# EmreAdabag/osqp

Measured on AMD Instinct MI355X. Metric: ADMM iters/sec (single QP), higher is better.
Workload: dtype f64; 1 GPU; config2 random sparse QP n=10000 m=20000 nnzA=200000 nnzPtriu=59985, one step = osqp_update_rho(0.1) + cold-started osqp_solve; adaptive_rho_interval=100, status=solved, graph_launches=4775, resident_gave_up=0, resident_slow_waits=0, parallelism=replicas x1 (a single QP does not shard)

## Files before the change

osqp_amd/csrc/engine.hip:

```cpp
#include <hip/hip_runtime.h>
#include <cstdio>
#include <new>
#include <cstdlib>
#include <cstring>
#include <cmath>
#include <vector>
#include <map>
#include <algorithm>
#include <mutex>
#include <condition_variable>
#include <thread>
#include <atomic>
#include <chrono>
#include "../../include/osqp_amd_engine.h"

#define TB 256
#define MAX_CHUNK 2048
#define LONG_ROW 512
#define HUGE_ROW 8192
#define MAX_PARTS 1024
#define MAX_HUGE_FOLD 4
#define INF_BOUND 1e26

#define HIPCHK(call)                                                            \
  do {                                                                          \
    hipError_t _e = (call);                                                     \
    if (_e != hipSuccess) {                                                     \
      fprintf(stderr, "osqp_amd: HIP error %s at %s:%d (%s)\n",                 \
              hipGetErrorString(_e), __FILE__, __LINE__, #call);                \
      return HIPENG_ERR_HIP;                                                    \
    }                                                                           \
  } while (0)

struct RowBlk { int r0, r1, k0, k1; };
#define IS_LONG(b) ((b).r1 - (b).r0 == 1 && (b).k1 - (b).k0 >= LONG_ROW)
struct __attribute__((aligned(32))) G4 { double r, w, s, m; };

struct DevMat {
  int nrows, nblk;
  int nstream;
  int nwave;
  const int    *rowptr;
  const int    *col;
  const unsigned short *col16;
  const double *val;
  const int    *split;
  const RowBlk *blk;
};

#define DENSE_MAX 128
struct DenseBlk { int c0, b, off, pitch; };
struct DenseP {
  int nblk;
  const DenseBlk *blk;
  const double *val;
};

struct State {
  int    run;
  int    done;
  int    stalled;
  int    neg_curv;
  int    iters[2];
  int    neg_curv_seen;
  int    iters_last;
  int    iters_max;
  int    iters_min;
  int    forced;
  long long iters_total;
  long long admm_done;
  double rz[2];
  double tol2;
  double gam[2], alp[2];
  int    hist_r;
  long long admm_target;
  unsigned res_epoch;
  int    res_fail;
  int    res_pipe_off;
  int    res_chk_fail;
  int    res_dbg[4];
  int    res_slow;
  int    res_slow_max;
  int    res_repub;
  int    res_slow_hist[4];
  unsigned res_slow_xcc;
  int    res_slow_last[4];
};

struct Params {
  double sigma, alpha, eps_rel, eps_abs, cinv;
  int    pcg_max_iter, use_cvec, has_scaling, pad0;
  double ex_theta;
  int    ex_h0, ex_h1;
  int    no_restart;
};

struct Ctx {
  int n, m;
  DevMat A, M;
  DevMat Mk;
  DenseP dP;
  int nh, hrow[MAX_HUGE_FOLD];
  const double *hcol;
  int gridA, gridM;
  double *xy, *z, *zt, *va, *vb, *q, *l, *u, *rho, *rhoinv, *minv, *pdiag;
  double *r, *zz, *kp, *pt0, *pt1, *dxy, *dy, *cvec;
  double *init_r, *init_z;
  double *vx, *vold;
  double *pdir, *ut;
  G4     *g4;
  int     init_stride;
  int     fin_wave_rows;
  double *vd;
  int     plain_rhs;
  const int *plain_skip;
  const unsigned short *u0map;
  double *u0pos;
  int     nelim;
  const int *erow, *ecol, *epos;
  double *rhoe, *ecoef, *edinv, *xte;
  double *D, *Dinv, *E, *Einv;
  double *part_rz, *part_rr, *part_bb, *part_pkp, *part_s0, *part_s1, *part_s2, *part_gam, *part_del;
  const double *fin_rr;
  int fin_cnt;
  double *scal;
  double *part_h;
  State  *st;
  const Params *prm;
#ifdef OSQP_AMD_TIMELINE
  unsigned long long *tl;
#endif
};

#ifdef OSQP_AMD_TIMELINE
#define TL_CAP (1 << 20)
#define TL_MARK(c, id) do { if (blockIdx.x == 0 && threadIdx.x == 0) { const unsigned long long k_ = atomicAdd((c).tl, 1ull); \
    if (k_ < TL_CAP - 2) (c).tl[1 + k_] = ((unsigned long long)(id) << 56) | (wall_clock64() & 0x00FFFFFFFFFFFFFFull); } } while (0)
#else
#define TL_MARK(c, id) do { } while (0)
#endif

enum {
  SC_PRI_U, SC_PRI_S, SC_Z_U, SC_Z_S, SC_AX_U, SC_AX_S,
  SC_DUA_U, SC_DUA_S, SC_Q_U, SC_Q_S, SC_ATY_U, SC_ATY_S, SC_PX_U, SC_PX_S,
  SC_DYN_U, SC_DYN_S, SC_DXN_U, SC_DXN_S,
  SC_ATDY_U, SC_ATDY_S, SC_PDX_U, SC_PDX_S, SC_ADX_VIOL,
  SC_OBJ, SC_DYLHS, SC_QDX,
  SC_COUNT
};
#define SCI(x) ((x) * 16)

template <int CTRL>
__device__ __forceinline__ double dpp_move(double v) {
  int lo = __double2loint(v), hi = __double2hiint(v);
  lo = __builtin_amdgcn_mov_dpp(lo, CTRL, 0xF, 0xF, true); hi = __builtin_amdgcn_mov_dpp(hi, CTRL, 0xF, 0xF, true);
  return __hiloint2double(hi, lo);
}
__device__ __forceinline__ double lane_value(double v, int lane) {
  return __hiloint2double(__builtin_amdgcn_readlane(__double2hiint(v), lane), __builtin_amdgcn_readlane(__double2loint(v), lane));
}
__device__ __forceinline__ double wave_sum(double v) {
  v += dpp_move<0xB1>(v); v += dpp_move<0x4E>(v); v += dpp_move<0x141>(v); v += dpp_move<0x140>(v);
  return (lane_value(v, 0) + lane_value(v, 16)) + (lane_value(v, 32) + lane_value(v, 48));
}

__device__ __forceinline__ double block_sum(double v, double *red) {
  v = wave_sum(v);
  const int lane = threadIdx.x & 63, w = threadIdx.x >> 6;
  __syncthreads();
  if (lane == 0) red[w] = v;
  __syncthreads();
  if (threadIdx.x == 0) red[4] = (red[0] + red[1]) + (red[2] + red[3]);
  __syncthreads();
  return red[4];
}

__device__ __forceinline__ void block_sum3(double &a, double &b, double &c, double *red) {
  a = wave_sum(a); b = wave_sum(b); c = wave_sum(c);
  const int lane = threadIdx.x & 63, w = threadIdx.x >> 6;
  __syncthreads();
  if (lane == 0) { red[w] = a; red[4 + w] = b; red[8 + w] = c; }
  __syncthreads();
  a = (red[0] + red[1]) + (red[2] + red[3]);
  b = (red[4] + red[5]) + (red[6] + red[7]);
  c = (red[8] + red[9]) + (red[10] + red[11]);
}

template <int NA>
__device__ __forceinline__ void reduce_parts(const double *a0, const double *a1,
                                             const double *a2, int count,
                                             double *red, double out[NA]) {
  double s0 = 0, s1 = 0, s2 = 0;
  for (int i = threadIdx.x; i < count; i += TB) {
    s0 += a0[i];
    if (NA > 1) s1 += a1[i];
    if (NA > 2) s2 += a2[i];
  }
  if (NA == 1) { out[0] = block_sum(s0, red); return; }
  block_sum3(s0, s1, s2, red);
  out[0] = s0; out[1] = s1;
  if (NA > 2) out[2] = s2;
}

__device__ __forceinline__ void atomic_max_pos(double *slot, double v) {
  atomicMax(reinterpret_cast<unsigned long long *>(slot),
            static_cast<unsigned long long>(__double_as_longlong(v)));
}

__device__ __forceinline__ void block_max_to(double v, double *slot, double *red) {
#pragma unroll
  for (int off = 32; off > 0; off >>= 1) v = fmax(v, __shfl_down(v, off, 64));
  const int lane = threadIdx.x & 63, w = threadIdx.x >> 6;
  __syncthreads();
  if (lane == 0) red[w] = v;
  __syncthreads();
  if (threadIdx.x == 0) atomic_max_pos(slot, fmax(fmax(red[0], red[1]), fmax(red[2], red[3])));
}

template <int NV>
__device__ __forceinline__ void stage_products(const DevMat &Mx, const RowBlk b,
                                               const double *in0, const double *in1,
                                               double *l0, double *l1) {
  constexpr int E = MAX_CHUNK / TB;
  const int cnt = b.k1 - b.k0;
  int cc[E]; double vv[E], x0[E], x1[E];
#pragma unroll
  for (int e = 0; e < E; ++e) {
    const int k = threadIdx.x + e * TB;
    if (k < cnt) { cc[e] = Mx.col[b.k0 + k]; vv[e] = Mx.val[b.k0 + k]; }
  }
#pragma unroll
  for (int e = 0; e < E; ++e) {
    const int k = threadIdx.x + e * TB;
    if (k < cnt) { x0[e] = in0[cc[e]]; if (NV == 2) x1[e] = in1[cc[e]]; }
  }
#pragma unroll
  for (int e = 0; e < E; ++e) {
    const int k = threadIdx.x + e * TB;
    if (k < cnt) { l0[k] = vv[e] * x0[e]; if (NV == 2) l1[k] = vv[e] * x1[e]; }
  }
}

__device__ __forceinline__ double row_sum(const double *l, int a, int b) {
  double s = 0.0;
  for (int k = a; k < b; ++k) s += l[k];
  return s;
}

__device__ __forceinline__ double row_sum_par(const double *l, int a, int b, int lane, int L) {
  double s = 0.0;
  for (int k = a + lane; k < b; k += L) s += l[k];
  if (L >= 2) s += dpp_move<0xB1>(s);
  if (L >= 4) s += dpp_move<0x4E>(s);
  if (L >= 8) s += dpp_move<0x141>(s);
  if (L >= 16) s += dpp_move<0x140>(s);
  if (L >= 32) s += __shfl_xor(s, 16, 64);
  if (L == 64) s += __shfl_xor(s, 32, 64);
  return s;
}
__device__ __forceinline__ int lanes_for(int nrows) {
  int L = 64;
  while (L > 1 && L * nrows > TB) L >>= 1;
  return L;
}

__device__ __forceinline__ double long_row_dot(const DevMat &Mx, int ka, int kb,
                                               const double *in, double *red) {
  double s0 = 0.0, s1 = 0.0, s2 = 0.0, s3 = 0.0;
  int k = ka + threadIdx.x;
  for (; k + 3 * TB < kb; k += 4 * TB) {
    const int c0 = Mx.col[k], c1 = Mx.col[k + TB], c2 = Mx.col[k + 2 * TB], c3 = Mx.col[k + 3 * TB];
    const double v0 = Mx.val[k], v1 = Mx.val[k + TB], v2 = Mx.val[k + 2 * TB], v3 = Mx.val[k + 3 * TB];
    s0 += v0 * in[c0]; s1 += v1 * in[c1]; s2 += v2 * in[c2]; s3 += v3 * in[c3];
  }
  for (; k < kb; k += TB) s0 += Mx.val[k] * in[Mx.col[k]];
  return block_sum((s0 + s1) + (s2 + s3), red);
}

#define ROW_U 12
template <bool NARROW, class F>
__device__ __forceinline__ double wave_row_dot_t(const DevMat &Mx, int ka, int kb, F xval) {
  const int lane = threadIdx.x & 63;
  double s0 = 0.0, s1 = 0.0, s2 = 0.0, s3 = 0.0;
  for (int k0 = ka + lane; k0 - lane < kb; k0 += 64 * ROW_U) {
    int cc[ROW_U]; double vv[ROW_U], xx[ROW_U];
#pragma unroll
    for (int q = 0; q < ROW_U; ++q) {
      const int kc = min(k0 + 64 * q, kb - 1);
      cc[q] = NARROW ? (int)Mx.col16[kc] : Mx.col[kc];
      vv[q] = Mx.val[kc];
    }
#pragma unroll
    for (int q = 0; q < ROW_U; ++q) xx[q] = xval(cc[q]);
#pragma unroll
    for (int q = 0; q < ROW_U; ++q) if (k0 + 64 * q >= kb) vv[q] = 0.0;
#pragma unroll
    for (int q = 0; q < ROW_U; q += 4) { s0 += vv[q] * xx[q]; s1 += vv[q + 1] * xx[q + 1]; s2 += vv[q + 2] * xx[q + 2]; s3 += vv[q + 3] * xx[q + 3]; }
  }
  return wave_sum((s0 + s1) + (s2 + s3));
}
template <class F>
__device__ __forceinline__ double wave_row_dot(const DevMat &Mx, int ka, int kb, F xval) {
  return Mx.col16 ? wave_row_dot_t<true>(Mx, ka, kb, xval) : wave_row_dot_t<false>(Mx, ka, kb, xval);
}

template <bool EARLY = false, class XL>
__device__ __forceinline__ double dense_block_mv_x(const DenseP &dP, const DenseBlk d, XL xload, double *scratch) {
  const int lane = threadIdx.x & 63, w = threadIdx.x >> 6;
  const double2 *dv = reinterpret_cast<const double2 *>(dP.val + d.off);
  const int hp = d.pitch >> 1;
  double xe = 0.0;
  if (EARLY) {
    if ((int)threadIdx.x < d.b) xe = xload(d.c0 + (int)threadIdx.x);
    asm volatile("s_waitcnt vmcnt(0)" ::: "memory");
  }
  double2 v[DENSE_MAX / 4];
#pragma unroll
  for (int q = 0; q < DENSE_MAX / 4; ++q) {
    const int j = w + 4 * q;
    v[q] = (j < d.b && lane < hp) ? dv[(size_t)j * hp + lane] : double2{0.0, 0.0};
  }
  double *xl = scratch + 4 * DENSE_MAX;
  if ((int)threadIdx.x < DENSE_MAX) xl[threadIdx.x] = EARLY ? xe : ((int)threadIdx.x < d.b ? xload(d.c0 + (int)threadIdx.x) : 0.0);
  __syncthreads();
  double a0 = 0.0, a1 = 0.0;
#pragma unroll
  for (int q = 0; q < DENSE_MAX / 4; ++q) {
    const double u = xl[min(w + 4 * q, DENSE_MAX - 1)];
    a0 += v[q].x * u; a1 += v[q].y * u;
  }
  scratch[w * DENSE_MAX + 2 * lane] = a0; scratch[w * DENSE_MAX + 2 * lane + 1] = a1;
  __syncthreads();
  const int r = threadIdx.x;
  return r < d.b ? (scratch[r] + scratch[DENSE_MAX + r]) + (scratch[2 * DENSE_MAX + r] + scratch[3 * DENSE_MAX + r]) : 0.0;
}
__device__ __forceinline__ double dense_block_mv(const DenseP &dP, const DenseBlk d, const double *x, double *scratch) {
  return dense_block_mv_x<false>(dP, d, [x](int j) { return x[j]; }, scratch);
}

#define LDS_DECL(NV)                                   \
  __shared__ double lprod[(NV) * MAX_CHUNK];           \
  __shared__ double red[16]


__global__ void __launch_bounds__(TB) k_vd(Ctx c) {
  for (int k = blockIdx.x * TB + threadIdx.x; k < c.n + c.m; k += gridDim.x * TB) c.vd[k] = c.vb[k] - c.vx[k];
}
template <bool DENSE>
__global__ void __launch_bounds__(TB) k_pcg_init(Ctx c, int bench) {
  State *st = c.st;
  TL_MARK(c, 1);
  if (!bench) {
    if (st->stalled || st->res_fail) return;
    if (st->admm_done >= st->admm_target) { if (blockIdx.x == 0 && threadIdx.x == 0) st->run = 0; return; }
  }
  LDS_DECL(2);
  const Params prm = *c.prm;
  double prz = 0, prr = 0, pbb = 0;
  const DevMat &Mm = DENSE ? c.Mk : c.M;
  if (DENSE)
  for (int db = blockIdx.x; db < c.dP.nblk; db += gridDim.x) {
    const DenseBlk d = c.dP.blk[db];
    double sA = c.plain_rhs ? 0.0 : dense_block_mv(c.dP, d, c.vx, lprod);
    if ((int)threadIdx.x < d.b) {
      const int j = d.c0 + threadIdx.x;
      double sB = 0.0;
      if (c.plain_rhs) {
        for (int k = Mm.rowptr[j]; k < Mm.rowptr[j + 1]; ++k) { const int cc = Mm.col[k]; if (c.plain_skip && c.plain_skip[cc - c.n] >= 0) continue; sB += Mm.val[k] * c.vb[cc]; }
      } else {
        for (int k = Mm.rowptr[j]; k < Mm.rowptr[j + 1]; ++k) { const int cc = Mm.col[k]; const double v = Mm.val[k]; sA += v * c.vx[cc]; sB += v * c.vb[cc]; }
        for (int k = 0; k < c.nh; ++k) { const double hc = c.hcol[(size_t)k * c.n + j]; sA += hc * c.vx[c.n + c.hrow[k]]; sB += hc * c.vb[c.n + c.hrow[k]]; }
      }
      const double base = prm.use_cvec ? c.cvec[j] : (prm.sigma * c.xy[j] - c.q[j]);
      const double bj = base + sB;
      const double rj = c.plain_rhs ? bj : bj - prm.sigma * c.vx[j] - sA;
      const double zj = c.minv[j] * rj;
      c.init_r[(size_t)j * c.init_stride] = rj;
      c.init_z[j] = zj;
      if (c.u0pos) c.u0pos[c.u0map[j]] = zj;
      prz += rj * zj; prr += rj * rj; pbb += bj * bj;
    }
    __syncthreads();
  }
  auto row_start = [&](int j, double sA, double sB) {
    if (DENSE) for (int k = 0; k < c.nh; ++k) { const double hc = c.hcol[(size_t)k * c.n + j]; sA += hc * c.vx[c.n + c.hrow[k]]; sB += hc * c.vb[c.n + c.hrow[k]]; }
    const double base = prm.use_cvec ? c.cvec[j] : (prm.sigma * c.xy[j] - c.q[j]);
    const bool gone = c.nelim && c.erow[j] >= 0;
    const double bj = gone ? 0.0 : base + sB;
    const double rj = gone ? 0.0 : bj - prm.sigma * c.vx[j] - sA;
    const double zj = c.minv[j] * rj;
    c.init_r[(size_t)j * c.init_stride] = rj;
    c.init_z[j] = zj;
    if (c.u0pos) c.u0pos[c.u0map[j]] = zj;
    prz += rj * zj; prr += rj * rj; pbb += bj * bj;
  };
  for (int bi = blockIdx.x; bi < Mm.nstream; bi += gridDim.x) {
    const RowBlk b = Mm.blk[bi];
    stage_products<2>(Mm, b, c.vx, c.vb, lprod, lprod + MAX_CHUNK);
    __syncthreads();
    const int RL = lanes_for(b.r1 - b.r0), rg = threadIdx.x / RL, rlane = threadIdx.x % RL;
    for (int j = b.r0 + rg; j < b.r1; j += TB / RL) {
      const int a0 = Mm.rowptr[j] - b.k0, a1 = Mm.rowptr[j + 1] - b.k0;
      const double sA = row_sum_par(lprod, a0, a1, rlane, RL);
      const double sB = row_sum_par(lprod + MAX_CHUNK, a0, a1, rlane, RL);
      if (rlane == 0) row_start(j, sA, sB);
    }
    __syncthreads();
  }
  for (int bi = Mm.nstream + blockIdx.x * (TB / 64) + (threadIdx.x >> 6); bi < Mm.nblk; bi += gridDim.x * (TB / 64)) {
    const RowBlk lb = Mm.blk[bi];
    const int lane = threadIdx.x & 63;
    if (c.vd) {
      const double acc = wave_row_dot(Mm, lb.k0, lb.k1, [&](int cc) { return c.vd[cc]; });
      if (lane == 0) row_start(lb.r0, -acc, 0.0);
      continue;
    }
    double a0 = 0.0, a1 = 0.0, b0 = 0.0, b1 = 0.0;
    const bool narrow = Mm.col16 != nullptr;
    constexpr int UI = 8;
    for (int k0 = lb.k0 + lane; k0 - lane < lb.k1; k0 += 64 * UI) {
      int cc[UI]; double vv[UI], xa[UI], xb[UI];
#pragma unroll
      for (int q = 0; q < UI; ++q) {
        const int kc = min(k0 + 64 * q, lb.k1 - 1);
        cc[q] = narrow ? (int)Mm.col16[kc] : Mm.col[kc];
        vv[q] = Mm.val[kc];
      }
#pragma unroll
      for (int q = 0; q < UI; ++q) { xa[q] = c.vx[cc[q]]; xb[q] = c.vb[cc[q]]; }
#pragma unroll
      for (int q = 0; q < UI; ++q) if (k0 + 64 * q >= lb.k1) vv[q] = 0.0;
#pragma unroll
      for (int q = 0; q < UI; q += 2) { a0 += vv[q] * xa[q]; b0 += vv[q] * xb[q]; a1 += vv[q + 1] * xa[q + 1]; b1 += vv[q + 1] * xb[q + 1]; }
    }
    const double sA = wave_sum(a0 + a1), sB = wave_sum(b0 + b1);
    if (lane == 0) row_start(lb.r0, sA, sB);
  }
  block_sum3(prz, prr, pbb, red);
  if (threadIdx.x == 0) {
    c.part_rz[blockIdx.x] = prz; c.part_rr[blockIdx.x] = prr; c.part_bb[blockIdx.x] = pbb;
    if (blockIdx.x == 0) {
      st->run = 1; st->done = 0; st->neg_curv = 0; st->iters[0] = 0; st->iters[1] = 0;
      if (st->hist_r < (1 << 20)) st->hist_r += 1;
    }
  }
}

#define EPT (MAX_CHUNK / TB)

struct CgStep { double alpha, beta; bool first, stop, conv, bad; };
__device__ __forceinline__ CgStep cg_step(double rr, double gam, double del, double gam_old, double alp_old,
                                          double tol2, int iters_prev, int neg, const Params &prm, bool bench) {
  CgStep s;
  s.first = gam_old == 0.0;
  s.bad = false;
  if (s.first) { s.beta = 0.0; s.alpha = gam / del; }
  else {
    s.beta = gam / gam_old;
    const double den = del - s.beta * gam / alp_old;
    if (!(den > 0.0) && del > 0.0) {
      if (!prm.no_restart && rr <= 1e8 * tol2) { s.first = true; s.beta = 0.0; s.alpha = gam / del; }
      else { s.alpha = gam / den; s.bad = true; }
    } else s.alpha = gam / den;
  }
  if (bench) { s.beta = 0.5; s.alpha = 1e-3; s.bad = false; }
  s.conv = rr <= tol2;
  s.bad = s.bad || !(s.alpha > 0.0) || !(del > 0.0);
  s.stop = !bench && (s.conv || iters_prev >= prm.pcg_max_iter || neg || s.bad);
  return s;
}
__global__ void __launch_bounds__(TB) k_cg_A(Ctx c, int it, int flags) {
  State *st = c.st;
  TL_MARK(c, 2);
  const bool bench = flags & 4, upd_only = flags & 16, apply_only = flags & 32;
  const bool pre = (flags & 8) || apply_only;
  if (!bench && it >= (flags >> 8) && (it >= st->iters_last || st->stalled) && (!st->run || st->done)) return;
  const int stalled = st->stalled, run = st->run, done = st->done, neg = st->neg_curv;
  const int iters_prev = st->iters[(it + 1) & 1];
  const double tol2_old = st->tol2, gam_old = st->gam[(it + 1) & 1], alp_old = st->alp[(it + 1) & 1];
  const Params prm = *c.prm;
  const bool has_blk = (int)blockIdx.x < c.A.nstream;
  RowBlk b = {0, 0, 0, 0};
  if (has_blk) b = c.A.blk[blockIdx.x];
  const int cnt = b.k1 - b.k0;
  const bool small = has_blk;
  const G4 *gold = c.g4 + (size_t)((it + 1) & 1) * c.n;
  G4 *gnew = c.g4 + (size_t)(it & 1) * c.n;
  int ecol[EPT]; double eval[EPT], g0[EPT], g1[EPT], g2[EPT], g3[EPT];
  int RL = lanes_for(b.r1 - b.r0);
  int rg = threadIdx.x / RL, rlane = threadIdx.x % RL;
  int rp0 = 0, rp1 = 0;
  double prho = 0.0;
  if (small) {
    if (b.r0 + rg < b.r1) { rp0 = c.A.rowptr[b.r0 + rg]; rp1 = c.A.rowptr[b.r0 + rg + 1]; prho = c.rhoe[b.r0 + rg]; }
#pragma unroll
    for (int e = 0; e < EPT; ++e) {
      const int k = threadIdx.x + e * TB;
      if (k < cnt) { ecol[e] = c.A.col[b.k0 + k]; eval[e] = c.A.val[b.k0 + k]; }
    }
#pragma unroll
    for (int e = 0; e < EPT; ++e) {
      const int k = threadIdx.x + e * TB;
      if (k < cnt) {
        const int cc = ecol[e];
        if (pre) g0[e] = c.ut[cc];
        else { const G4 g = gold[cc]; g0[e] = g.r; g1[e] = g.w; g2[e] = g.s; g3[e] = g.m; }
      }
    }
  }
  double q0 = 0, q1 = 0, q2 = 0;
  if (!apply_only) {
    const double *a1 = pre ? c.part_bb : c.part_gam;
    for (int i = threadIdx.x; i < c.gridM; i += TB) { q0 += c.part_rr[i]; q1 += a1[i]; if (!pre) q2 += c.part_del[i]; }
  }
  const int j0 = blockIdx.x * TB + threadIdx.x;
  double o_u = 0, o_w = 0, o_p = 0, o_s = 0, o_r = 0, o_x = 0, o_m = 0;
  if (!pre && j0 < c.n) {
    const G4 g = gold[j0];
    o_u = c.ut[j0]; o_w = g.w; o_p = c.pdir[j0]; o_s = g.s; o_r = g.r; o_x = gam_old == 0.0 ? c.vx[j0] : c.va[j0]; o_m = g.m;
  }
  if (!bench && (!run || done || ((flags & 8) && stalled))) return;
  LDS_DECL(1);
  double sums[3];
  bool first = false;
  double alpha = 0.0, beta = 0.0, tol2 = tol2_old;
  sums[0] = q0; sums[1] = q1; sums[2] = q2;
  if (!apply_only) block_sum3(sums[0], sums[1], sums[2], red);
  if (apply_only) {
  } else if (pre) {
    tol2 = fmax(prm.eps_rel * prm.eps_rel * sums[1], prm.eps_abs * prm.eps_abs);
    if (!bench && sums[0] <= tol2) {
      if (blockIdx.x == 0 && threadIdx.x == 0) { st->done = 1; st->tol2 = tol2; }
      return;
    }
    if (blockIdx.x == 0 && threadIdx.x == 0) { st->tol2 = tol2; st->gam[1] = 0.0; st->alp[1] = 0.0; }
  } else {
    const double gam = sums[1];
    const bool fresh = gam_old == 0.0;
    const CgStep cs = cg_step(sums[0], gam, sums[2], gam_old, alp_old, tol2, iters_prev, neg, prm, bench);
    first = cs.first; alpha = cs.alpha; beta = cs.beta;
    if (cs.stop) {
      if (blockIdx.x == 0 && threadIdx.x == 0) { st->done = cs.conv ? 1 : 2; if (cs.bad && !cs.conv) st->neg_curv = 1; }
      return;
    }
    if (blockIdx.x == 0 && threadIdx.x == 0) {
      st->gam[it & 1] = gam; st->alp[it & 1] = alpha; st->iters[it & 1] = iters_prev + 1;
    }
    for (int j = j0; j < c.n; j += gridDim.x * TB) {
      double uj, wj, po, so, ro, xo, mi;
      if (j == j0) { uj = o_u; wj = o_w; po = o_p; so = o_s; ro = o_r; xo = o_x; mi = o_m; }
      else { const G4 g = gold[j]; uj = c.ut[j]; wj = g.w; po = c.pdir[j]; so = g.s; ro = g.r; xo = fresh ? c.vx[j] : c.va[j]; mi = g.m; }
      const double pj = first ? uj : (uj + beta * po);
      const double sj = first ? wj : (wj + beta * so);
      const double rj = ro - alpha * sj;
      c.pdir[j] = pj; gnew[j].s = sj; gnew[j].r = rj;
      c.va[j] = xo + alpha * pj;
      c.ut[j] = mi * rj;
    }
  }
  if (upd_only) return;
  double *t = c.ut + c.n;
  for (int bi = blockIdx.x; bi < c.A.nstream; bi += gridDim.x) {
    if (bi != (int)blockIdx.x) { b = c.A.blk[bi]; RL = lanes_for(b.r1 - b.r0); rg = threadIdx.x / RL; rlane = threadIdx.x % RL; }
    const int cn = b.k1 - b.k0;
    if (bi != (int)blockIdx.x) {
#pragma unroll
      for (int e = 0; e < EPT; ++e) {
        const int k = threadIdx.x + e * TB;
        if (k < cn) { ecol[e] = c.A.col[b.k0 + k]; eval[e] = c.A.val[b.k0 + k]; }
      }
#pragma unroll
      for (int e = 0; e < EPT; ++e) {
        const int k = threadIdx.x + e * TB;
        if (k < cn) {
          const int cc = ecol[e];
          if (pre) g0[e] = c.ut[cc];
          else { const G4 g = gold[cc]; g0[e] = g.r; g1[e] = g.w; g2[e] = g.s; g3[e] = g.m; }
        }
      }
    }
#pragma unroll
    for (int e = 0; e < EPT; ++e) {
      const int k = threadIdx.x + e * TB;
      if (k < cn) {
        double uv;
        if (pre) uv = g0[e];
        else {
          const double sj = first ? g1[e] : (g1[e] + beta * g2[e]);
          uv = g3[e] * (g0[e] - alpha * sj);
        }
        lprod[k] = eval[e] * uv;
      }
    }
    __syncthreads();
    for (int i = b.r0 + rg; i < b.r1; i += TB / RL) {
      int a0, a1;
      if (bi == (int)blockIdx.x && i == b.r0 + rg) { a0 = rp0; a1 = rp1; }
      else { a0 = c.A.rowptr[i]; a1 = c.A.rowptr[i + 1]; }
// ... 46 lines not shown
  s = block_sum(s, red);
  if (threadIdx.x == 0) c.ut[c.n + row] = c.rhoe[row] * s;
}

template <bool DENSE, bool FOLD>
__global__ void __launch_bounds__(TB) k_cg_B(Ctx c, int it, int flags) {
  State *st = c.st;
  TL_MARK(c, 3);
  const bool bench = flags & 4;
  if (!bench && it >= (flags >> 8) && (it >= st->iters_last || st->stalled) && (!st->run || st->done)) return;
  const int run = st->run, done = st->done, skip_pre = it < 0 && st->stalled;
  const double sigma = c.prm->sigma;
  const bool has_blk = (int)blockIdx.x < c.Mk.nstream;
  RowBlk b = {0, 0, 0, 0};
  if (has_blk) b = c.Mk.blk[blockIdx.x];
  const int cnt = b.k1 - b.k0;
  const bool small = has_blk;
  double ev[EPT];
  int RL = lanes_for(b.r1 - b.r0);
  int rg = threadIdx.x / RL, rlane = threadIdx.x % RL;
  int rp0 = 0, rp1 = 0;
  G4 *gc = c.g4 + (size_t)(it & 1) * c.n;
  double pu = 0.0, pr = 0.0;
  double hs[MAX_HUGE_FOLD], ph[MAX_HUGE_FOLD], hrho[MAX_HUGE_FOLD];
#pragma unroll
  for (int k = 0; k < MAX_HUGE_FOLD; ++k) {
    hs[k] = 0.0; ph[k] = 0.0; hrho[k] = 0.0;
    if (FOLD && k < c.nh) {
      hrho[k] = c.rhoe[c.hrow[k]];
      for (int i = threadIdx.x; i < c.gridA; i += TB) hs[k] += c.part_h[(size_t)k * c.gridA + i];
    }
  }
  if (small) {
    if (b.r0 + rg < b.r1) {
      rp0 = c.Mk.rowptr[b.r0 + rg]; rp1 = c.Mk.rowptr[b.r0 + rg + 1];
      pu = c.ut[b.r0 + rg]; pr = gc[b.r0 + rg].r;
#pragma unroll
      for (int k = 0; k < MAX_HUGE_FOLD; ++k) if (FOLD && k < c.nh) ph[k] = c.hcol[(size_t)k * c.n + b.r0 + rg];
    }
    int ecol[EPT];
#pragma unroll
    for (int e = 0; e < EPT; ++e) {
      const int k = threadIdx.x + e * TB;
      if (k < cnt) { ecol[e] = c.Mk.col[b.k0 + k]; ev[e] = c.Mk.val[b.k0 + k]; }
    }
#pragma unroll
    for (int e = 0; e < EPT; ++e) {
      const int k = threadIdx.x + e * TB;
      if (k < cnt) ev[e] = ev[e] * c.ut[ecol[e]];
    }
  }
  if (!bench && (!run || done || skip_pre)) return;
  LDS_DECL(1);
  double th[MAX_HUGE_FOLD];
#pragma unroll
  for (int k = 0; k < MAX_HUGE_FOLD; ++k) th[k] = (FOLD && k < c.nh) ? hrho[k] * block_sum(hs[k], red) : 0.0;
  auto hterm = [&](int j, bool pref) {
    double s = 0.0;
    if (FOLD) {
#pragma unroll
      for (int k = 0; k < MAX_HUGE_FOLD; ++k) if (k < c.nh) s += (pref ? ph[k] : c.hcol[(size_t)k * c.n + j]) * th[k];
    }
    return s;
  };
  double pg = 0, pd = 0, prr = 0;
  for (int bi = blockIdx.x; bi < c.Mk.nstream; bi += gridDim.x) {
    if (bi != (int)blockIdx.x) { b = c.Mk.blk[bi]; RL = lanes_for(b.r1 - b.r0); rg = threadIdx.x / RL; rlane = threadIdx.x % RL; }
    const int cn = b.k1 - b.k0;
    if (bi == (int)blockIdx.x) {
#pragma unroll
      for (int e = 0; e < EPT; ++e) { const int k = threadIdx.x + e * TB; if (k < cn) lprod[k] = ev[e]; }
    } else stage_products<1>(c.Mk, b, c.ut, nullptr, lprod, nullptr);
    __syncthreads();
    for (int j = b.r0 + rg; j < b.r1; j += TB / RL) {
      int a0, a1;
      if (bi == (int)blockIdx.x && j == b.r0 + rg) { a0 = rp0; a1 = rp1; }
      else { a0 = c.Mk.rowptr[j]; a1 = c.Mk.rowptr[j + 1]; }
      const double acc = row_sum_par(lprod, a0 - b.k0, a1 - b.k0, rlane, RL);
      if (rlane == 0) {
        const bool first = bi == (int)blockIdx.x && j == b.r0 + rg;
        const double uj = first ? pu : c.ut[j], rj = first ? pr : gc[j].r;
        const double wj = (c.nelim && c.erow[j] >= 0) ? 0.0 : (acc + sigma * uj) + hterm(j, first);
        gc[j].w = wj;
        pg += rj * uj; pd += wj * uj; prr += rj * rj;
      }
    }
    __syncthreads();
  }
  for (int bi = c.Mk.nstream + blockIdx.x * (TB / 64) + (threadIdx.x >> 6); bi < c.Mk.nblk; bi += gridDim.x * (TB / 64)) {
    const RowBlk lb = c.Mk.blk[bi];
    const double acc = wave_row_dot(c.Mk, lb.k0, lb.k1, [&](int cc) { return c.ut[cc]; });
    if ((threadIdx.x & 63) == 0) {
      const int j = lb.r0;
      const double uj = c.ut[j], wj = (acc + sigma * uj) + hterm(j, false), rj = gc[j].r;
      gc[j].w = wj; pg += rj * uj; pd += wj * uj; prr += rj * rj;
    }
  }
  if (DENSE)
  for (int db = blockIdx.x; db < c.dP.nblk; db += gridDim.x) {
    const DenseBlk d = c.dP.blk[db];
    double acc = dense_block_mv(c.dP, d, c.ut, lprod);
    if ((int)threadIdx.x < d.b) {
      const int jrow = d.c0 + threadIdx.x;
      for (int k = c.Mk.rowptr[jrow]; k < c.Mk.rowptr[jrow + 1]; ++k) acc += c.Mk.val[k] * c.ut[c.Mk.col[k]];
      const double uj = lprod[4 * DENSE_MAX + threadIdx.x], wj = (acc + sigma * uj) + hterm(jrow, false), rj = gc[jrow].r;
      gc[jrow].w = wj; pg += rj * uj; pd += wj * uj; prr += rj * rj;
    }
    __syncthreads();
  }
  block_sum3(pg, pd, prr, red);
  if (threadIdx.x == 0) { c.part_gam[blockIdx.x] = pg; c.part_del[blockIdx.x] = pd; c.part_rr[blockIdx.x] = prr; }
}


__global__ void __launch_bounds__(TB) k_huge_dot(Ctx c, const double *x, int always) {
  if (!always && !c.st->run) return;
  if (!x) {
    const State *st = c.st;
    x = (c.vx != c.va && st->iters[0] == 0 && st->iters[1] == 0) ? c.vx : c.va;
  }
  __shared__ double red[16];
  for (int bi = c.A.nwave; bi < c.A.nblk; ++bi) {
    const RowBlk hb = c.A.blk[bi];
    double s0 = 0.0, s1 = 0.0;
    int k = hb.k0 + blockIdx.x * TB + threadIdx.x;
    const int stride = gridDim.x * TB;
    for (; k + stride < hb.k1; k += 2 * stride) {
      const int c0 = c.A.col[k], c1 = c.A.col[k + stride];
      s0 += c.A.val[k] * x[c0]; s1 += c.A.val[k + stride] * x[c1];
    }
    if (k < hb.k1) s0 += c.A.val[k] * x[c.A.col[k]];
    const double tot = block_sum(s0 + s1, red);
    if (threadIdx.x == 0) c.part_h[(size_t)(bi - c.A.nwave) * gridDim.x + blockIdx.x] = tot;
  }
}
__device__ __forceinline__ double huge_row_sum(const Ctx &c, int bi, double *red) {
  const double *part = c.part_h + (size_t)(bi - c.A.nwave) * c.gridA;
  double s = 0.0;
  for (int i = threadIdx.x; i < c.gridA; i += TB) s += part[i];
  return block_sum(s, red);
}

__device__ __forceinline__ double elim_vb(const Ctx &c, const Params &prm, int i, double rho, double vbn, double x_y) {
  const int y = c.ecol[i];
  if (y < 0) return vbn;
  const double a = c.ecoef[i];
  const double by = (prm.use_cvec ? c.cvec[y] : (prm.sigma * x_y - c.q[y])) + a * vbn;
  return vbn - rho * a * by * c.edinv[i];
}

__global__ void __launch_bounds__(TB) k_admm_finalize(Ctx c) {
  State *st = c.st;
  TL_MARK(c, 4);
  if (!st->run || st->res_fail) return;
  LDS_DECL(1);
  const Params prm = *c.prm;
  double rr[1];
  reduce_parts<1>(c.fin_rr, nullptr, nullptr, c.fin_cnt, red, rr);
  const int iters = st->iters[0] > st->iters[1] ? st->iters[0] : st->iters[1];
  const bool conv = st->done == 1 || rr[0] <= st->tol2;
  const bool force = st->done == 2 || iters >= prm.pcg_max_iter || st->neg_curv;
  if (!conv && !force) {
    if (blockIdx.x == 0 && threadIdx.x == 0) st->stalled = 1;
    return;
  }
  if (blockIdx.x == 0 && threadIdx.x == 0) {
    st->stalled = 0;
    st->admm_done += 1;
    st->iters_last = iters;
    st->iters_total += iters;
    if (iters > st->iters_max) st->iters_max = iters;
    if (iters < st->iters_min) st->iters_min = iters;
    if (!conv) st->forced += 1;
    if (st->neg_curv) st->neg_curv_seen += 1;
  }
  const double alpha = prm.alpha, oma = 1.0 - prm.alpha;
  const int hist = st->hist_r;
  const double th = (hist < prm.ex_h0 ? 0.0 : (hist < prm.ex_h1 ? 0.5 : 1.0)) * prm.ex_theta;
  const bool ex = c.vx != c.va;
  const bool from_start = ex && iters == 0;
  const double *xts = from_start ? c.vx : c.va;
  double *x = c.xy, *y = c.xy + c.n;
  for (int j = blockIdx.x * TB + threadIdx.x; j < c.n; j += gridDim.x * TB) {
    if (c.nelim && c.erow[j] >= 0) continue;
    const double xo = x[j], xt = xts[j];
    const double xn = alpha * xt + oma * xo;
    c.dxy[j] = xn - xo;
    x[j] = xn;
    if (ex) { c.vx[j] = xt + th * (xt - c.vold[j]); c.vold[j] = xt; }
    if (from_start) c.va[j] = xt;
  }
  auto row_update = [&](int i, double zt) {
    const double rho = c.rho[i], rinv = c.rhoinv[i], yo = y[i], zo = c.z[i];
    const int ye = c.nelim ? c.ecol[i] : -1;
    double rz = rho * zt, xny = 0.0;
    if (ye >= 0) {
      const double a = c.ecoef[i], xoy = x[ye];
      const double by = (prm.use_cvec ? c.cvec[ye] : (prm.sigma * xoy - c.q[ye])) + a * (rho * zo - yo);
      const double xty = (by - rho * a * zt) * c.edinv[i];
      rz = c.rhoe[i] * zt;
      zt += a * xty;
      xny = alpha * xty + oma * xoy;
      c.dxy[ye] = xny - xoy; x[ye] = xny; c.xte[i] = xty;
    }
    double v = alpha * zt + oma * zo + rinv * yo;
    v = fmax(v, c.l[i]);
    const double zn = fmin(v, c.u[i]);
    const double dy = rho * (alpha * zt + oma * zo - zn);
    const double yn = yo + dy;
    c.z[i] = zn; y[i] = yn; c.dy[i] = dy; c.zt[i] = zt;
    c.va[c.n + i] = rz;
    if (ex) { c.vx[c.n + i] = rz + th * (rz - c.vold[c.n + i]); c.vold[c.n + i] = rz; }
    c.vb[c.n + i] = ye >= 0 ? elim_vb(c, prm, i, rho, rho * zn - yn, xny) : rho * zn - yn;
  };
  for (int bi = blockIdx.x; bi < c.A.nstream; bi += gridDim.x) {
    const RowBlk b = c.A.blk[bi];
    stage_products<1>(c.A, b, xts, nullptr, lprod, nullptr);
    __syncthreads();
    const int RL = lanes_for(b.r1 - b.r0), rg = threadIdx.x / RL, rlane = threadIdx.x % RL;
    for (int i = b.r0 + rg; i < b.r1; i += TB / RL) {
      const double zt = row_sum_par(lprod, c.A.rowptr[i] - b.k0, c.A.rowptr[i + 1] - b.k0, rlane, RL);
      if (rlane == 0) row_update(i, zt);
    }
    __syncthreads();
  }
  if (c.fin_wave_rows) {
    const int lane = threadIdx.x & 63, wv = threadIdx.x >> 6;
    for (int bi = c.A.nstream + blockIdx.x * (TB / 64) + wv; bi < c.A.nwave; bi += gridDim.x * (TB / 64)) {
      const RowBlk lb = c.A.blk[bi];
      const double zt = wave_row_dot(c.A, lb.k0, lb.k1, [&](int cc) { return xts[cc]; });
      if (lane == 0) row_update(lb.r0, zt);
    }
  } else
  for (int bi = c.A.nstream + blockIdx.x; bi < c.A.nwave; bi += gridDim.x) {
    const RowBlk lb = c.A.blk[bi];
    const double zt = long_row_dot(c.A, lb.k0, lb.k1, xts, red);
    if (threadIdx.x == 0) row_update(lb.r0, zt);
    __syncthreads();
  }
  for (int bi = c.A.nwave + blockIdx.x; bi < c.A.nblk; bi += gridDim.x) {
    const double zt = huge_row_sum(c, bi, red);
    if (threadIdx.x == 0) row_update(c.A.blk[bi].r0, zt);
    __syncthreads();
  }
}


#define RES_TB 512
#define RES_PT (RES_TB - 64)
#define RES_MAXROWS 61
#define RES_MAXN (RES_MAXROWS * 256)
#define RES_MAXPAD 16384
#define RES_MAXLD (RES_MAXPAD / 2 / RES_TB)
#define RES_WAIT_TICKS 2000000LL
#define RES_SLOW_TICKS 5000LL
#define AUX_SC1 16
#define AUX_VOL ((int)0x80000000)
#define RES_DBG 16
#define RES_FSTRIDE 32
#define RES_GSTRIDE 16
typedef unsigned int u32x4 __attribute__((ext_vector_type(4)));
typedef unsigned int u32x2 __attribute__((ext_vector_type(2)));
struct ResWG { int r0, nr, cnt, pos; };
struct ResCtx {
  int nwg, E, npad;
  int npw;
  const unsigned short *rowpos;
  int pipe;
  int u0_direct;
  int inject;
  const ResWG *wg;
  double *val;
  const unsigned short *col;
  const unsigned char *rowl;
  const int *krp, *kcj, *kps, *kdst;
  const unsigned long long *brk;
  const unsigned short *slot0;
  const unsigned short *segrow;
  double *ubuf;
  unsigned *flags;
  int *dbg;
  double *sbuf;
};

static __device__ __forceinline__ __amdgpu_buffer_rsrc_t res_rsrc(const void *p, size_t bytes) {
  return __builtin_amdgcn_make_buffer_rsrc(const_cast<void *>(p), 0, (int)bytes, 0x00020000);
}

__device__ __forceinline__ int res_spin_check(State *st, long long &t0, int &late) {
  const long long now = wall_clock64();
  const long long el = now - t0;
  if (el < 0 || el > (1LL << 40)) { t0 = now; late = 0; return 0; }
  if (__hip_atomic_load(&st->res_fail, __ATOMIC_RELAXED, __HIP_MEMORY_SCOPE_AGENT)) return 2;
  if (el > RES_WAIT_TICKS) { if (late) return 1; late = 1; } else late = 0;
  return 0;
}
__device__ __forceinline__ void res_note(State *st, int *dbg, int g, int verdict, int kind, int nx, int first, unsigned seen, long long t0, unsigned rounds, int gidx) {
  if (verdict == 1 && atomicCAS(&st->res_dbg[0], 0, kind) == 0) { st->res_dbg[1] = nx; st->res_dbg[2] = g; st->res_dbg[3] = first; }
  int *d = dbg + (size_t)RES_DBG * g;
  const long long now = wall_clock64();
  d[3] = verdict == 1 ? kind : 3; d[4] = first; d[5] = (int)seen; d[6] = (int)(now - t0);
  d[7] = (int)__builtin_amdgcn_s_getreg((3 << 11) | 20);
  d[8] = (int)(unsigned)now; d[9] = (int)rounds; d[10] = gidx;
}
__device__ __forceinline__ void res_slow_note(State *st, long long t0, int nx, int g, int missed, int kind) {
  const long long el = wall_clock64() - t0;
  if (el > RES_SLOW_TICKS && el < (1LL << 40)) {
    atomicAdd(&st->res_slow, 1); atomicMax(&st->res_slow_max, (int)(el > 0x7fffffffLL ? 0x7fffffffLL : el));
    atomicAdd(&st->res_slow_hist[el < 20000 ? 0 : (el < 50000 ? 1 : (el < 200000 ? 2 : 3))], 1);
    atomicOr(&st->res_slow_xcc, 1u << (__builtin_amdgcn_s_getreg((3 << 11) | 20) & 15));
    st->res_slow_last[0] = nx; st->res_slow_last[1] = g; st->res_slow_last[2] = missed; st->res_slow_last[3] = kind;
  }
}

__device__ __forceinline__ int lane_int(int v, int l) { return __builtin_amdgcn_readlane(v, l); }
__global__ void __launch_bounds__(TB) k_form_K(Ctx c, ResCtx rc) {
  const double sigma = c.prm->sigma;
  if (blockIdx.x == 0 && threadIdx.x == 0) c.st->res_pipe_off = 0;
  const int lane = threadIdx.x & 63, nwaves = gridDim.x * (TB / 64);
  for (int i = blockIdx.x * (TB / 64) + (threadIdx.x >> 6); i < c.n; i += nwaves) {
    const int e0 = rc.krp[i], e1 = rc.krp[i + 1];
    const int ka = c.M.split[i], kb = c.M.rowptr[i + 1];
    for (int eb = e0; eb < e1; eb += 256) {
      int j[4]; double v[4];
#pragma unroll
      for (int q = 0; q < 4; ++q) {
        const int idx = eb + q * 64 + lane;
        j[q] = -1; v[q] = 0.0;
        if (idx < e1) {
          j[q] = rc.kcj[idx];
          const int ps = rc.kps[idx];
          v[q] = (ps >= 0 ? c.M.val[ps] : 0.0) + (j[q] == i ? sigma : 0.0);
        }
      }
      for (int kc = ka; kc < kb; kc += 64) {
        const bool on = kc + lane < kb;
        const int kk = on ? c.M.col[kc + lane] - c.n : 0;
        const double ai = on ? c.M.val[kc + lane] : 0.0, rk = on ? c.rhoe[kk] : 0.0;
        const int p0 = on ? c.A.rowptr[kk] : 0, p1 = on ? c.A.rowptr[kk + 1] : 0;
        const int cnt = min(64, kb - kc);
        for (int q = 0; q < cnt; ++q) {
          const double a_i = lane_value(ai, q), r = lane_value(rk, q);
          const int s0 = lane_int(p0, q), s1 = lane_int(p1, q);
          for (int ec = s0; ec < s1; ec += 64) {
            const bool eon = ec + lane < s1;
            const int cj = eon ? c.A.col[ec + lane] : -1;
            const double av = eon ? c.A.val[ec + lane] : 0.0;
            const int len = min(64, s1 - ec);
            for (int e = 0; e < len; ++e) {
              const int cjb = lane_int(cj, e);
              const double t = r * (a_i * lane_value(av, e));
#pragma unroll
              for (int q4 = 0; q4 < 4; ++q4) if (j[q4] == cjb) v[q4] += t;
            }
          }
        }
      }
      const bool igone = c.nelim && c.erow[i] >= 0;
#pragma unroll
      for (int q = 0; q < 4; ++q) {
        const int idx = eb + q * 64 + lane;
        if (idx < e1) {
          const bool gone = c.nelim && (igone || c.erow[j[q]] >= 0);
          rc.val[rc.kdst[idx]] = gone ? (j[q] == i ? 1.0 : 0.0) : v[q];
        }
      }
    }
  }
}

template <int E>
__global__ void __launch_bounds__(RES_TB) k_pcg_resident(Ctx c, ResCtx rc) {
  extern __shared__ __attribute__((aligned(16))) double rlds[];
  State *st = c.st;
  TL_MARK(c, 5);
  if (st->stalled || !st->run || st->res_fail) return;
  double *uv = rlds;
  double *seg = uv + rc.npad;
  double *sc = seg + RES_TB + RES_MAXROWS;
  double *sval = sc + 8;
#ifdef OSQP_AMD_TIMELINE
  long long *tls = reinterpret_cast<long long *>(sval + 768);
#define RTL(k) do { if (blockIdx.x == 0 && threadIdx.x == 0 && nx >= 1 && nx <= 64) tls[(nx - 1) * 5 + (k)] = wall_clock64(); } while (0)
  long long *wtl = tls + 5 * 64;
#define WTL(k) do { if (blockIdx.x == 0 && (threadIdx.x & 63) == 0 && (nx == 8 || nx == 1)) wtl[(nx == 1 ? 40 : 0) + (k) * 8 + (threadIdx.x >> 6)] = wall_clock64(); } while (0)
  if (blockIdx.x == 0 && threadIdx.x == 0) wtl[80] = wall_clock64();
#else
#define RTL(k) do { } while (0)
#define WTL(k) do { } while (0)
#endif
  const int g = blockIdx.x, t = threadIdx.x, lane = t & 63, wv = t >> 6;
  const int nwg = rc.nwg, npad = rc.npad;
  const ResWG w = rc.wg[g];
  const Params prm = *c.prm;
  const unsigned ep0 = st->res_epoch;
  const bool sabotage = rc.inject > 0 && g == rc.nwg - 1 && st->admm_done + 1 == rc.inject;
  bool pipe = rc.pipe && !st->res_pipe_off && !prm.no_restart;
// ... 2931 lines not shown
```

Before: 7774 ADMM iters/s.

## Prefetch first row block and state before early-exit checks in PCG init/finalize

In k_pcg_init and k_admm_finalize, each block now issues its loads up front, before the early-exit checks and the global state reads resolve. These loads cover the state fields, the first streaming row block's column indices and values, the row pointers, the per-row inputs and the fin_rr partials. The first block's products and row updates then use these registers, which hides global-memory latency at kernel start. It also adds timeline instrumentation macros that compile away by default. In exchange, loads are wasted when the kernel exits early, register pressure rises, and there is a subtle change: vx is no longer written in the from_start case.

```diff
diff --git a/osqp_amd/csrc/engine.hip b/osqp_amd/csrc/engine.hip
--- a/osqp_amd/csrc/engine.hip
+++ b/osqp_amd/csrc/engine.hip
@@ -136,8 +136,20 @@
 #define TL_CAP (1 << 20)
 #define TL_MARK(c, id) do { if (blockIdx.x == 0 && threadIdx.x == 0) { const unsigned long long k_ = atomicAdd((c).tl, 1ull); \
     if (k_ < TL_CAP - 2) (c).tl[1 + k_] = ((unsigned long long)(id) << 56) | (wall_clock64() & 0x00FFFFFFFFFFFFFFull); } } while (0)
+#define TLK_N 10
+#define TLK_DECL long long tlk_[TLK_N], tll_[2] = {0, 0}; for (int q_ = 0; q_ < TLK_N; ++q_) tlk_[q_] = 0
+#define TLK_LAST(k) do { if (k) asm volatile("s_waitcnt vmcnt(0)" ::: "memory"); if (blockIdx.x == gridDim.x - 1 && threadIdx.x == 0) tll_[k] = wall_clock64(); } while (0)
+#define TLK_AT(k, v) do { asm volatile("" :: "v"(v)); if (blockIdx.x == 0 && threadIdx.x == 0) tlk_[k] = wall_clock64(); } while (0)
+#define TLK_FLUSH(c, base, n) do { if (blockIdx.x == 0 && threadIdx.x == 0) { const unsigned long long k_ = atomicAdd((c).tl, (unsigned long long)(n)); \
+    if (k_ + (n) < TL_CAP - 2) for (int q_ = 0; q_ < (n); ++q_) (c).tl[1 + k_ + q_] = ((unsigned long long)((base) + q_) << 56) | ((unsigned long long)tlk_[q_] & 0x00FFFFFFFFFFFFFFull); } \
+  if (blockIdx.x == gridDim.x - 1 && threadIdx.x == 0) { const unsigned long long k_ = atomicAdd((c).tl, 2ull); \
+    if (k_ + 2 < TL_CAP - 2) for (int q_ = 0; q_ < 2; ++q_) (c).tl[1 + k_ + q_] = ((unsigned long long)((base) + 20 + q_) << 56) | ((unsigned long long)tll_[q_] & 0x00FFFFFFFFFFFFFFull); } } while (0)
 #else
 #define TL_MARK(c, id) do { } while (0)
+#define TLK_DECL do { } while (0)
+#define TLK_AT(k, v) do { } while (0)
+#define TLK_LAST(k) do { } while (0)
+#define TLK_FLUSH(c, base, n) do { } while (0)
 #endif
 
 enum {
@@ -350,14 +362,50 @@
 __global__ void __launch_bounds__(TB) k_pcg_init(Ctx c, int bench) {
   State *st = c.st;
   TL_MARK(c, 1);
+  TLK_DECL;
+  TLK_AT(0, 0); TLK_LAST(0);
+  LDS_DECL(2);
+  const DevMat &Mm = DENSE ? c.Mk : c.M;
+  const int s_stalled = st->stalled, s_fail = st->res_fail, s_hist = st->hist_r;
+  const long long s_admm = st->admm_done, s_target = st->admm_target;
+  const Params prm = *c.prm;
+  RowBlk b = RowBlk{0, 0, 0, 0};
+  if constexpr (!DENSE) {
+    b = Mm.blk[max(min((int)blockIdx.x, Mm.nstream - 1), 0)];
+    if ((int)blockIdx.x >= Mm.nstream) b = RowBlk{0, 0, 0, 0};
+  }
+  TLK_AT(1, b.k1);
+  struct RowIn { double base0, base1, vx, minv; int u0, er; };
+  const unsigned short *u0m = c.u0pos ? c.u0map : reinterpret_cast<const unsigned short *>(c.minv);
+  const int *erw = c.nelim ? c.erow : reinterpret_cast<const int *>(c.minv);
+  auto row_load = [&](int j) {
+    RowIn r;
+    r.base0 = (prm.use_cvec ? c.cvec : c.xy)[j]; r.base1 = c.q[j];
+    r.vx = c.vx[j]; r.minv = c.minv[j];
+    r.u0 = (int)u0m[j]; r.er = erw[j];
+    return r;
+  };
+  constexpr int E = MAX_CHUNK / TB;
+  const int cnt = b.k1 - b.k0;
+  int cc[E] = {}; double vv[E] = {};
+  const int RL = lanes_for(b.r1 - b.r0), rg = threadIdx.x / RL, rlane = threadIdx.x % RL;
+  const int jf = b.r0 + rg, jfc = max(min(jf, b.r1 - 1), 0);
+  int p0 = 0, p1 = 0;
+  RowIn rf = {};
+  if constexpr (!DENSE) {
+#pragma unroll
+    for (int e = 0; e < E; ++e) {
+      const int kc = max(min(b.k0 + (int)threadIdx.x + e * TB, b.k1 - 1), 0);
+      cc[e] = Mm.col[kc]; vv[e] = Mm.val[kc];
+    }
+    p0 = Mm.rowptr[jfc]; p1 = Mm.rowptr[jfc + 1];
+    rf = row_load(jfc);
+  }
   if (!bench) {
-    if (st->stalled || st->res_fail) return;
-    if (st->admm_done >= st->admm_target) { if (blockIdx.x == 0 && threadIdx.x == 0) st->run = 0; return; }
-  }
-  LDS_DECL(2);
-  const Params prm = *c.prm;
+    if (s_stalled || s_fail) return;
+    if (s_admm >= s_target) { if (blockIdx.x == 0 && threadIdx.x == 0) st->run = 0; return; }
+  }
   double prz = 0, prr = 0, pbb = 0;
-  const DevMat &Mm = DENSE ? c.Mk : c.M;
   if (DENSE)
   for (int db = blockIdx.x; db < c.dP.nblk; db += gridDim.x) {
     const DenseBlk d = c.dP.blk[db];
@@ -382,28 +430,53 @@
     }
     __syncthreads();
   }
-  auto row_start = [&](int j, double sA, double sB) {
+  auto row_apply = [&](int j, double sA, double sB, const RowIn &r) {
     if (DENSE) for (int k = 0; k < c.nh; ++k) { const double hc = c.hcol[(size_t)k * c.n + j]; sA += hc * c.vx[c.n + c.hrow[k]]; sB += hc * c.vb[c.n + c.hrow[k]]; }
-    const double base = prm.use_cvec ? c.cvec[j] : (prm.sigma * c.xy[j] - c.q[j]);
-    const bool gone = c.nelim && c.erow[j] >= 0;
+    const double base = prm.use_cvec ? r.base0 : (prm.sigma * r.base0 - r.base1);
+    const bool gone = c.nelim && r.er >= 0;
     const double bj = gone ? 0.0 : base + sB;
-    const double rj = gone ? 0.0 : bj - prm.sigma * c.vx[j] - sA;
-    const double zj = c.minv[j] * rj;
+    const double rj = gone ? 0.0 : bj - prm.sigma * r.vx - sA;
+    const double zj = r.minv * rj;
     c.init_r[(size_t)j * c.init_stride] = rj;
     c.init_z[j] = zj;
-    if (c.u0pos) c.u0pos[c.u0map[j]] = zj;
+    if (c.u0pos) c.u0pos[r.u0] = zj;
     prz += rj * zj; prr += rj * rj; pbb += bj * bj;
   };
-  for (int bi = blockIdx.x; bi < Mm.nstream; bi += gridDim.x) {
-    const RowBlk b = Mm.blk[bi];
-    stage_products<2>(Mm, b, c.vx, c.vb, lprod, lprod + MAX_CHUNK);
+  auto row_start = [&](int j, double sA, double sB) { row_apply(j, sA, sB, row_load(j)); };
+  if (!DENSE) {
+    double xa[E], xb[E];
+    TLK_AT(2, cc[E - 1]);
+#pragma unroll
+    for (int e = 0; e < E; ++e) { xa[e] = c.vx[cc[e]]; xb[e] = c.vb[cc[e]]; }
+    TLK_AT(3, xb[E - 1]);
+#pragma unroll
+    for (int e = 0; e < E; ++e) { const int k = threadIdx.x + e * TB; if (k < cnt) { lprod[k] = vv[e] * xa[e]; lprod[MAX_CHUNK + k] = vv[e] * xb[e]; } }
     __syncthreads();
-    const int RL = lanes_for(b.r1 - b.r0), rg = threadIdx.x / RL, rlane = threadIdx.x % RL;
-    for (int j = b.r0 + rg; j < b.r1; j += TB / RL) {
+    TLK_AT(4, 0);
+    if (jf < b.r1) {
+      const double sA = row_sum_par(lprod, p0 - b.k0, p1 - b.k0, rlane, RL);
+      const double sB = row_sum_par(lprod + MAX_CHUNK, p0 - b.k0, p1 - b.k0, rlane, RL);
+      if (rlane == 0) row_apply(jf, sA, sB, rf);
+    }
+    TLK_AT(5, prz);
+    for (int j = jf + TB / RL; j < b.r1; j += TB / RL) {
       const int a0 = Mm.rowptr[j] - b.k0, a1 = Mm.rowptr[j + 1] - b.k0;
       const double sA = row_sum_par(lprod, a0, a1, rlane, RL);
       const double sB = row_sum_par(lprod + MAX_CHUNK, a0, a1, rlane, RL);
       if (rlane == 0) row_start(j, sA, sB);
+    }
+    __syncthreads();
+  }
+  for (int bi = DENSE ? blockIdx.x : blockIdx.x + gridDim.x; bi < Mm.nstream; bi += gridDim.x) {
+    const RowBlk bb = Mm.blk[bi];
+    stage_products<2>(Mm, bb, c.vx, c.vb, lprod, lprod + MAX_CHUNK);
+    __syncthreads();
+    const int RLb = lanes_for(bb.r1 - bb.r0), rgb = threadIdx.x / RLb, rlb = threadIdx.x % RLb;
+    for (int j = bb.r0 + rgb; j < bb.r1; j += TB / RLb) {
+      const int a0 = Mm.rowptr[j] - bb.k0, a1 = Mm.rowptr[j + 1] - bb.k0;
+      const double sA = row_sum_par(lprod, a0, a1, rlb, RLb);
+      const double sB = row_sum_par(lprod + MAX_CHUNK, a0, a1, rlb, RLb);
+      if (rlb == 0) row_start(j, sA, sB);
     }
     __syncthreads();
   }
@@ -437,13 +510,16 @@
     if (lane == 0) row_start(lb.r0, sA, sB);
   }
   block_sum3(prz, prr, pbb, red);
+  TLK_AT(6, prz);
   if (threadIdx.x == 0) {
     c.part_rz[blockIdx.x] = prz; c.part_rr[blockIdx.x] = prr; c.part_bb[blockIdx.x] = pbb;
     if (blockIdx.x == 0) {
       st->run = 1; st->done = 0; st->neg_curv = 0; st->iters[0] = 0; st->iters[1] = 0;
-      if (st->hist_r < (1 << 20)) st->hist_r += 1;
-    }
-  }
+      if (s_hist < (1 << 20)) st->hist_r = s_hist + 1;
+    }
+  }
+  TLK_LAST(1);
+  TLK_FLUSH(c, 100, 7);
 }
 
 #define EPT (MAX_CHUNK / TB)
@@ -796,75 +872,147 @@
 __global__ void __launch_bounds__(TB) k_admm_finalize(Ctx c) {
   State *st = c.st;
   TL_MARK(c, 4);
-  if (!st->run || st->res_fail) return;
+  TLK_DECL;
+  TLK_AT(0, 0); TLK_LAST(0);
   LDS_DECL(1);
+  const int s_run = st->run, s_fail = st->res_fail, s_done = st->done, s_neg = st->neg_curv, s_hist = st->hist_r;
+  const int s_it0 = st->iters[0], s_it1 = st->iters[1];
+  const double s_tol2 = st->tol2;
+  const long long s_admm = st->admm_done, s_total = st->iters_total;
+  const int s_max = st->iters_max, s_min = st->iters_min, s_forced = st->forced, s_negseen = st->neg_curv_seen;
   const Params prm = *c.prm;
-  double rr[1];
-  reduce_parts<1>(c.fin_rr, nullptr, nullptr, c.fin_cnt, red, rr);
-  const int iters = st->iters[0] > st->iters[1] ? st->iters[0] : st->iters[1];
-  const bool conv = st->done == 1 || rr[0] <= st->tol2;
-  const bool force = st->done == 2 || iters >= prm.pcg_max_iter || st->neg_curv;
+  const bool ex = c.vx != c.va;
+  const bool have = (int)blockIdx.x < c.A.nstream;
+  RowBlk b = c.A.blk[max(min((int)blockIdx.x, c.A.nstream - 1), 0)];
+  if (!have) b = RowBlk{0, 0, 0, 0};
+  TLK_AT(1, b.k1);
+  constexpr int NP = MAX_PARTS / TB;
+  double fp[NP];
+#pragma unroll
+  for (int k = 0; k < NP; ++k) fp[k] = c.fin_rr[max(min((int)threadIdx.x + k * TB, c.fin_cnt - 1), 0)];
+  double *x = c.xy, *y = c.xy + c.n;
+  const int j0 = blockIdx.x * TB + threadIdx.x, jc = max(min(j0, c.n - 1), 0);
+  const double xo0 = x[jc], xa0 = c.va[jc], xv0 = c.vx[jc], vo0 = c.vold[jc];
+  struct RowIn { double rho, rinv, yo, zo, lo, up, vo, ea, edi, rhe; int ye; };
+  auto row_load = [&](int i) {
+    RowIn r;
+    r.rho = c.rho[i]; r.rinv = c.rhoinv[i]; r.yo = y[i]; r.zo = c.z[i]; r.lo = c.l[i]; r.up = c.u[i];
+    r.vo = c.vold[c.n + i];
+    r.ye = -1; r.ea = 0.0; r.edi = 0.0; r.rhe = 0.0;
+    if (c.nelim) { r.ye = c.ecol[i]; r.ea = c.ecoef[i]; r.edi = c.edinv[i]; r.rhe = c.rhoe[i]; }
+    return r;
+  };
+  constexpr int E = MAX_CHUNK / TB;
+  const int cnt = b.k1 - b.k0;
+  int cc[E]; double vv[E];
+#pragma unroll
+  for (int e = 0; e < E; ++e) {
+    const int kc = max(min(b.k0 + (int)threadIdx.x + e * TB, b.k1 - 1), 0);
+    cc[e] = c.A.col[kc]; vv[e] = c.A.val[kc];
+  }
+  const int RL = lanes_for(b.r1 - b.r0), rg = threadIdx.x / RL, rlane = threadIdx.x % RL;
+  const int i0 = b.r0 + rg, ic = max(min(i0, b.r1 - 1), 0);
+  const int p0 = c.A.rowptr[ic], p1 = c.A.rowptr[min(ic + 1, c.A.nrows)];
+  const RowIn ri0 = row_load(ic);
+  const int er0 = (c.nelim ? c.erow : reinterpret_cast<const int *>(c.rho))[c.nelim ? jc : 0];
+  TLK_AT(2, fp[NP - 1]);
+  if (!s_run || s_fail) return;
+  double rr[1] = {0.0};
+  if (s_done != 1) {
+    double s0 = 0;
+#pragma unroll
+    for (int k = 0; k < NP; ++k) s0 = (int)threadIdx.x + k * TB < c.fin_cnt ? s0 + fp[k] : s0;
+    for (int i = threadIdx.x + NP * TB; i < c.fin_cnt; i += TB) s0 += c.fin_rr[i];
+    rr[0] = block_sum(s0, red);
+  }
+  TLK_AT(3, rr[0]);
+  const int iters = s_it0 > s_it1 ? s_it0 : s_it1;
+  const bool conv = s_done == 1 || rr[0] <= s_tol2;
+  const bool force = s_done == 2 || iters >= prm.pcg_max_iter || s_neg;
   if (!conv && !force) {
     if (blockIdx.x == 0 && threadIdx.x == 0) st->stalled = 1;
     return;
   }
   if (blockIdx.x == 0 && threadIdx.x == 0) {
     st->stalled = 0;
-    st->admm_done += 1;
+    st->admm_done = s_admm + 1;
     st->iters_last = iters;
-    st->iters_total += iters;
-    if (iters > st->iters_max) st->iters_max = iters;
-    if (iters < st->iters_min) st->iters_min = iters;
-    if (!conv) st->forced += 1;
-    if (st->neg_curv) st->neg_curv_seen += 1;
+    st->iters_total = s_total + iters;
+    if (iters > s_max) st->iters_max = iters;
+    if (iters < s_min) st->iters_min = iters;
+    if (!conv) st->forced = s_forced + 1;
+    if (s_neg) st->neg_curv_seen = s_negseen + 1;
   }
   const double alpha = prm.alpha, oma = 1.0 - prm.alpha;
-  const int hist = st->hist_r;
+  const int hist = s_hist;
   const double th = (hist < prm.ex_h0 ? 0.0 : (hist < prm.ex_h1 ? 0.5 : 1.0)) * prm.ex_theta;
-  const bool ex = c.vx != c.va;
   const bool from_start = ex && iters == 0;
   const double *xts = from_start ? c.vx : c.va;
-  double *x = c.xy, *y = c.xy + c.n;
-  for (int j = blockIdx.x * TB + threadIdx.x; j < c.n; j += gridDim.x * TB) {
-    if (c.nelim && c.erow[j] >= 0) continue;
-    const double xo = x[j], xt = xts[j];
+  auto x_update = [&](int j, double xo, double xt, double vo) {
     const double xn = alpha * xt + oma * xo;
     c.dxy[j] = xn - xo;
     x[j] = xn;
-    if (ex) { c.vx[j] = xt + th * (xt - c.vold[j]); c.vold[j] = xt; }
+    if (ex) { if (!from_start) c.vx[j] = xt + th * (xt - vo); c.vold[j] = xt; }
     if (from_start) c.va[j] = xt;
-  }
-  auto row_update = [&](int i, double zt) {
-    const double rho = c.rho[i], rinv = c.rhoinv[i], yo = y[i], zo = c.z[i];
-    const int ye = c.nelim ? c.ecol[i] : -1;
+  };
+  if (j0 < c.n && !(c.nelim && er0 >= 0)) x_update(j0, xo0, from_start ? xv0 : xa0, vo0);
+  for (int j = j0 + gridDim.x * TB; j < c.n; j += gridDim.x * TB) {
+    if (c.nelim && c.erow[j] >= 0) continue;
+    x_update(j, x[j], xts[j], c.vold[j]);
+  }
+  auto row_apply = [&](int i, double zt, const RowIn &r) {
+    const double rho = r.rho, rinv = r.rinv, yo = r.yo, zo = r.zo;
+    const int ye = r.ye;
     double rz = rho * zt, xny = 0.0;
     if (ye >= 0) {
-      const double a = c.ecoef[i], xoy = x[ye];
+      const double a = r.ea, xoy = x[ye];
       const double by = (prm.use_cvec ? c.cvec[ye] : (prm.sigma * xoy - c.q[ye])) + a * (rho * zo - yo);
-      const double xty = (by - rho * a * zt) * c.edinv[i];
-      rz = c.rhoe[i] * zt;
+      const double xty = (by - rho * a * zt) * r.edi;
+      rz = r.rhe * zt;
       zt += a * xty;
       xny = alpha * xty + oma * xoy;
       c.dxy[ye] = xny - xoy; x[ye] = xny; c.xte[i] = xty;
     }
     double v = alpha * zt + oma * zo + rinv * yo;
-    v = fmax(v, c.l[i]);
-    const double zn = fmin(v, c.u[i]);
+    v = fmax(v, r.lo);
+    const double zn = fmin(v, r.up);
     const double dy = rho * (alpha * zt + oma * zo - zn);
     const double yn = yo + dy;
     c.z[i] = zn; y[i] = yn; c.dy[i] = dy; c.zt[i] = zt;
     c.va[c.n + i] = rz;
-    if (ex) { c.vx[c.n + i] = rz + th * (rz - c.vold[c.n + i]); c.vold[c.n + i] = rz; }
+    if (ex) { c.vx[c.n + i] = rz + th * (rz - r.vo); c.vold[c.n + i] = rz; }
     c.vb[c.n + i] = ye >= 0 ? elim_vb(c, prm, i, rho, rho * zn - yn, xny) : rho * zn - yn;
   };
-  for (int bi = blockIdx.x; bi < c.A.nstream; bi += gridDim.x) {
-    const RowBlk b = c.A.blk[bi];
-    stage_products<1>(c.A, b, xts, nullptr, lprod, nullptr);
+  auto row_update = [&](int i, double zt) { row_apply(i, zt, row_load(i)); };
+  {
+    double xg[E];
+    TLK_AT(4, cc[E - 1]);
+#pragma unroll
+    for (int e = 0; e < E; ++e) xg[e] = xts[cc[e]];
+    TLK_AT(5, xg[E - 1]);
+#pragma unroll
+    for (int e = 0; e < E; ++e) { const int k = threadIdx.x + e * TB; if (k < cnt) lprod[k] = vv[e] * xg[e]; }
     __syncthreads();
-    const int RL = lanes_for(b.r1 - b.r0), rg = threadIdx.x / RL, rlane = threadIdx.x % RL;
-    for (int i = b.r0 + rg; i < b.r1; i += TB / RL) {
+    TLK_AT(6, 0);
+    if (i0 < b.r1) {
+      const double zt = row_sum_par(lprod, p0 - b.k0, p1 - b.k0, rlane, RL);
+      if (rlane == 0) row_apply(i0, zt, ri0);
+    }
+    TLK_AT(7, 0);
+    for (int i = i0 + TB / RL; i < b.r1; i += TB / RL) {
       const double zt = row_sum_par(lprod, c.A.rowptr[i] - b.k0, c.A.rowptr[i + 1] - b.k0, rlane, RL);
       if (rlane == 0) row_update(i, zt);
+    }
+    __syncthreads();
+  }
+  for (int bi = blockIdx.x + gridDim.x; bi < c.A.nstream; bi += gridDim.x) {
+    const RowBlk bb = c.A.blk[bi];
+    stage_products<1>(c.A, bb, xts, nullptr, lprod, nullptr);
+    __syncthreads();
+    const int RLb = lanes_for(bb.r1 - bb.r0), rgb = threadIdx.x / RLb, rlb = threadIdx.x % RLb;
+    for (int i = bb.r0 + rgb; i < bb.r1; i += TB / RLb) {
+      const double zt = row_sum_par(lprod, c.A.rowptr[i] - bb.k0, c.A.rowptr[i + 1] - bb.k0, rlb, RLb);
+      if (rlb == 0) row_update(i, zt);
     }
     __syncthreads();
   }
@@ -887,6 +1035,8 @@
     if (threadIdx.x == 0) row_update(c.A.blk[bi].r0, zt);
     __syncthreads();
   }
+  TLK_AT(8, 0); TLK_LAST(1);
+  TLK_FLUSH(c, 110, 9);
 }
 
 
```

After: 7949 ADMM iters/s, median of 6. 1.02x the previous value.
